# 20k/geodesic_raytracing

Measured on AMD Instinct MI355X. Metric: Mrays/sec at 3840x2160 Kerr (whole frame: prepass + init + adaptive Verlet + render-data + anisotropic render), higher is better.
Workload: dtype f32; 1 GPU; kerr_boyer (Boyer-Lindquist rs=1 a=0.45) 3840x2160, camera (0,0,-4,0) fov 90, adaptive_sampling off, prepass on, tol 1e-06, background 4096x2048 RGBA8 10 mips, anisotropy 8; mode=fused, prepass_lookahead=True, prepass_lookahead_depth=1, frames_in_flight=3, prepass=look-ahead on side streams, priming_frames=0, build_key=c7636d8b88329620-v80s8, counters_tag=kerr_a045_4k, program=substituted (parameters baked in, metric_manager.hpp:153-166), parallelism=single GPU

## Files before the change

### geodesic_raytracing_amd/__init__.py

```python
import ctypes
import os

_HERE = os.path.dirname(os.path.abspath(__file__))
LIB_PATH = os.path.join(_HERE, "libgeodesic_hip.so")

if not os.path.exists(LIB_PATH):
    raise ImportError(
        f"{LIB_PATH} is missing: build it with `python -c 'import __graft_entry__ as g; g.build()'` "
        "(there is no CPU fallback for the ray kernels)")

lib = ctypes.CDLL(LIB_PATH)

c_void_p = ctypes.c_void_p
c_int = ctypes.c_int
c_float = ctypes.c_float
c_char_p = ctypes.c_char_p
c_size_t = ctypes.c_size_t


class Features(ctypes.Structure):
    _fields_ = [
        ("adaptive_sampling_threshold", c_float), ("field_of_view", c_float), ("max_acceleration_change", c_float),
        ("max_precision_radius", c_float), ("min_step", c_float), ("ray_skip", c_float), ("universe_size", c_float),
        ("adaptive_sampling", c_int), ("redshift", c_int), ("reparameterisation", c_int), ("use_old_redshift", c_int),
# ... 64 lines not shown
                ("block_rows", c_int), ("strip_rank", c_int), ("strip_count", c_int), ("termination_buffer", c_void_p),
                ("prepass_width", c_int), ("prepass_height", c_int), ("e0", c_void_p), ("e1", c_void_p), ("e2", c_void_p),
                ("e3", c_void_p), ("cfg", c_void_p), ("dfg", c_void_p), ("attempt_counter", c_void_p), ("tile_order", c_void_p),
                ("waves_per_simd", c_int), ("shading", TraceShading), ("lattice", c_int), ("pending_only", c_int), ("inline_prepass", c_int),
                ("tile_cost", c_void_p), ("tile_order_by_history", c_int), ("lattice_rays", c_void_p), ("parking", ParkingLot), ("speculative_classes", c_int), ("guessed", c_void_p)]


class Transport(ctypes.Structure):
    GROUP = ctypes.CFUNCTYPE(c_int, c_void_p)
    SEND = ctypes.CFUNCTYPE(c_int, c_void_p, c_void_p, c_size_t, c_int, c_void_p)
    RECV = ctypes.CFUNCTYPE(c_int, c_void_p, c_void_p, c_size_t, c_int, c_void_p)
    _fields_ = [("user", c_void_p), ("group_begin", GROUP), ("group_end", GROUP), ("send", SEND), ("recv", RECV)]


MODE_REFERENCE, MODE_FUSED = 0, 1
EVAL_METRIC_TENSOR, EVAL_METRIC_DERIVATIVES, EVAL_ACCELERATION, EVAL_TO_POLAR, EVAL_FROM_POLAR, EVAL_ORIGIN_DISTANCE = range(6)
(STAGE_CAMERA, STAGE_PREPASS, STAGE_INIT, STAGE_TRACE, STAGE_RENDER_DATA, STAGE_ADAPTIVE, STAGE_RENDER) = range(7)
STAGE_NAMES = ["camera", "prepass", "init", "trace", "render_data", "adaptive", "render"]
(BUF_RAYS_IN, BUF_RAYS_COUNT, BUF_RENDER_DATA, BUF_TERMINATION, BUF_CAMERA_GENERIC, BUF_TETRAD0, BUF_TETRAD1, BUF_TETRAD2,
 BUF_TETRAD3, BUF_RAYS_ADAPTIVE, BUF_RAYS_ADAPTIVE_COUNT, BUF_CFG, BUF_DFG, BUF_CAMERA_QUAT) = range(14)

_SIGNATURES = {
    "gr_last_error": (c_char_p, []),
    "gr_features_default": (None, [ctypes.POINTER(Features)]),
    "gr_metric_builtin": (c_int, [c_char_p, ctypes.POINTER(c_void_p)]),
    "gr_metric_load_script": (c_int, [c_char_p, c_char_p, ctypes.POINTER(c_void_p)]),
    "gr_metric_from_info": (c_int, [ctypes.POINTER(MetricInfo), ctypes.POINTER(c_char_p), ctypes.POINTER(c_float), ctypes.POINTER(c_void_p)]),
    "gr_metric_destroy": (None, [c_void_p]),
    "gr_metric_get_info": (c_int, [c_void_p, ctypes.POINTER(MetricInfo)]),
    "gr_metric_dynamic_var_name": (c_char_p, [c_void_p, c_int]),
    "gr_metric_dynamic_var_default": (c_float, [c_void_p, c_int]),
    "gr_metric_argument_string": (c_int, [c_void_p, ctypes.POINTER(Features), c_int, ctypes.POINTER(c_float), c_int,
                                          c_char_p, c_size_t, ctypes.POINTER(c_size_t)]),
    "gr_metric_substituted_op_counts": (c_int, [c_void_p, ctypes.POINTER(c_float), c_int, ctypes.POINTER(c_int), ctypes.POINTER(c_int),
                                                ctypes.POINTER(c_int)]),
    "gr_metric_evaluate_count": (c_int, [c_int]),
    "gr_metric_evaluate": (c_int, [c_void_p, c_int, ctypes.POINTER(ctypes.c_double), ctypes.POINTER(ctypes.c_double), ctypes.POINTER(c_float), c_int,
                                   ctypes.POINTER(ctypes.c_double), c_int]),
    "gr_program_create": (c_int, [c_char_p, c_int, ctypes.POINTER(c_void_p)]),
    "gr_program_complete": (c_int, [c_void_p]),
    "gr_program_precompile_frame_path": (c_int, [c_char_p]),
    "gr_program_precompile": (c_int, [c_char_p]),
    "gr_program_create_async": (c_int, [c_char_p, c_int, ctypes.POINTER(c_void_p)]),
    "gr_program_future_poll": (c_int, [c_void_p, ctypes.POINTER(c_void_p)]),
    "gr_program_future_destroy": (None, [c_void_p]),
    "gr_program_destroy": (None, [c_void_p]),
    "gr_program_manager_create": (c_int, [c_void_p, c_int, ctypes.POINTER(Features), ctypes.POINTER(c_float), c_int, ctypes.POINTER(c_void_p)]),
    "gr_program_manager_update": (c_int, [c_void_p, ctypes.POINTER(Features), ctypes.POINTER(c_float), c_int]),
    "gr_program_manager_current": (c_int, [c_void_p, c_int, ctypes.POINTER(c_void_p), ctypes.POINTER(c_int)]),
    "gr_program_manager_dynamic": (c_void_p, [c_void_p]),
    "gr_program_manager_destroy": (None, [c_void_p]),
    "gr_do_generic_rays_scheduled": (c_int, [c_void_p, c_void_p, c_void_p, c_void_p, c_int, c_void_p, c_void_p, c_void_p, c_void_p, c_void_p]),
    "gr_sort_tiles_by_cost": (c_int, [c_void_p, c_void_p, c_void_p, c_int, c_int, c_void_p, c_void_p]),
    "gr_program_manager_counters": (None, [c_void_p, ctypes.POINTER(ctypes.c_ulonglong)]),
    "gr_program_kernel_info": (c_int, [c_void_p, c_char_p, ctypes.POINTER(c_int), ctypes.POINTER(c_int), ctypes.POINTER(c_int)]),
    "gr_cart_to_generic": (c_int, [c_void_p, c_void_p, c_void_p, c_void_p, c_int, c_float, c_void_p]),
    "gr_init_basis_vectors": (c_int, [c_void_p, c_void_p, c_void_p, c_int, ctypes.POINTER(c_float), c_void_p, c_void_p,
                                      c_void_p, c_void_p, c_void_p]),
    "gr_clear_termination_buffer": (c_int, [c_void_p, c_void_p, c_void_p, c_int, c_int]),
    "gr_init_rays_generic": (c_int, [c_void_p, c_void_p, c_void_p, c_void_p, c_void_p, c_void_p, c_int, c_int, c_void_p, c_int,
                                     c_int, c_int, c_void_p, c_void_p, c_void_p, c_void_p, c_void_p, c_void_p, c_int, c_int]),
    "gr_tiled_slot_count": (c_int, [c_int, c_int]),
    "gr_do_generic_rays": (c_int, [c_void_p, c_void_p, c_void_p, c_void_p, c_int, c_void_p, c_void_p, c_void_p, c_void_p, c_int,
                                   c_int, c_int, c_int, c_void_p, c_void_p, c_int, c_void_p]),
    "gr_calculate_singularities": (c_int, [c_void_p, c_void_p, c_void_p, c_void_p, c_int, c_void_p, c_int, c_int]),
    "gr_calculate_render_data": (c_int, [c_void_p, c_void_p, c_void_p, c_void_p, c_int, c_void_p, c_void_p, c_int, c_int,
# ... 134 lines not shown
```

### geodesic_raytracing_amd/csrc/capi.cpp

```cpp
#include "../../include/geodesic_hip_internal.h"

#include <dlfcn.h>
#include <hip/hip_runtime_api.h>
#include <hip/hiprtc.h>
#include <sys/stat.h>
#include <unistd.h>

#include <chrono>
#include <cmath>
#include <cstdio>
#include <algorithm>
#include <atomic>
#include <cstdlib>
#include <cstring>
#include <fstream>
#include <map>
#include <memory>
#include <condition_variable>
#include <mutex>
#include <sstream>
#include <string>
#include <system_error>
#include <thread>
#include <vector>
// ... 669 lines not shown
        env[vel_names[i]] = velocity ? velocity[i] : 0.0;
    }
    for (size_t i = 0; i < m->vars.names.size(); i++)
        env["cfg->" + m->vars.names[i]] = cfg_values ? (double)cfg_values[i] : (double)m->vars.defaults[i];
    env["always_lightlike"] = 0.0;
    const gr::MetricImpl& impl = m->desc.raw;
    auto eval_all = [&](const std::vector<sym::E>& v, double* dst) { for (size_t i = 0; i < v.size(); i++) dst[i] = sym::eval(v[i], env); };
    switch (what) {
        case GR_EVAL_METRIC_TENSOR:
            for (int i = 0; i < 16; i++) out[i] = 0.0;
            if (impl.real_eq.size() == 4) { for (int i = 0; i < 4; i++) out[i * 4 + i] = sym::eval(impl.real_eq[(size_t)i], env); }
            else eval_all(impl.real_eq, out);
            break;
        case GR_EVAL_METRIC_DERIVATIVES:
            for (int i = 0; i < 64; i++) out[i] = 0.0;
            if (impl.derivatives.size() == 16) { for (int k = 0; k < 4; k++) for (int i = 0; i < 4; i++) out[k * 16 + i * 4 + i] = sym::eval(impl.derivatives[(size_t)(k * 4 + i)], env); }
            else eval_all(impl.derivatives, out);
            break;
        case GR_EVAL_ACCELERATION: eval_all(impl.accel, out); break;
        case GR_EVAL_TO_POLAR: eval_all(impl.to_polar, out); break;
        case GR_EVAL_FROM_POLAR: eval_all(impl.from_polar, out); break;
        case GR_EVAL_ORIGIN_DISTANCE: {
            double polar[4];
            eval_all(impl.to_polar, polar);
            for (int i = 0; i < 4; i++) env[pos_names[i]] = polar[i];
            out[0] = sym::eval(impl.distance_function, env);
            break;
        }
    }
    return GR_OK;
    GR_TRY_END
}

int gr_metric_substituted_op_counts(const gr_metric* m, const float* cfg_values, int num_cfg_values, int* accel_ops,
                                    int* accel_transcendentals, int* coord_ops) {
    if (!m) return fail(GR_ERROR_INVALID_ARGUMENT, "null metric");
    if (m->settings_only) return fail(GR_ERROR_INVALID_ARGUMENT, "a metric made by gr_metric_from_info has no expressions to count");
    GR_TRY_BEGIN
    std::vector<float> vals(cfg_values, cfg_values + (cfg_values ? num_cfg_values : 0));
    const gr::MetricImpl concrete = m->desc.concrete(m->vars.substitution(vals));
    const sym::OpCount accel = sym::count_ops(concrete.accel);
    std::vector<sym::E> coord = concrete.to_polar;
    coord.push_back(concrete.distance_function);
    if (accel_ops) *accel_ops = accel.ops;
    if (accel_transcendentals) *accel_transcendentals = accel.transcendental;
    if (coord_ops) *coord_ops = sym::count_ops(coord).ops;
    return GR_OK;
    GR_TRY_END
}

int gr_argument_string_accelerations_call_trig(const char* argument_string) {
    if (!argument_string) return -1;
    std::vector<std::string> opts;
    for (auto& tok : split_arguments(argument_string))
        if (tok.rfind("-D", 0) == 0) opts.push_back(tok);
    return accelerations_without_trig(opts) ? 0 : 1;
}

int gr_program_precompile(const char* argument_string) {
    if (!argument_string) return fail(GR_ERROR_INVALID_ARGUMENT, "null argument string");
    std::string code, rest, setup;
    int rc = compile_code_object(argument_string, code);
    if (rc != GR_OK) return rc;
    rc = compile_code_object(argument_string, rest, nullptr, PART_REST);
    if (rc != GR_OK) return rc;
    return compile_setup_module(argument_string, setup);
// ... 990 lines not shown
```

### geodesic_raytracing_amd/csrc/metric_codegen.cpp

```cpp
#include <functional>
#include <unordered_set>
#include "metric_codegen.hpp"

#include <cmath>
#include <cstdio>
#include <cstring>
#include <sstream>
#include <iomanip>
#include <stdexcept>

using namespace sym;

namespace gr {


static bool parse_bool(const std::string& v) { return v == "true" || v == "1"; }

void MetricConfig::apply(const std::map<std::string, std::string>& kv) {
    for (auto& [key, value] : kv) {
        if (key == "name") name = value;
        else if (key == "description") description = value;
        else if (key == "use_prepass") use_prepass = parse_bool(value);
        else if (key == "max_acceleration_change") max_acceleration_change = std::stof(value);
        else if (key == "singular") singular = parse_bool(value);
        else if (key == "traversable_event_horizon") traversable_event_horizon = parse_bool(value);
        else if (key == "singular_terminator") singular_terminator = std::stof(value);
        else if (key == "adaptive_precision") adaptive_precision = parse_bool(value);
        else if (key == "detect_singularities") detect_singularities = parse_bool(value);
        else if (key == "follow_geodesics_forward") follow_geodesics_forward = parse_bool(value);
        else if (key == "coordinate_system") {
            if (value == "X_Y_THETA_PHI") system = CoordinateSystem::X_Y_THETA_PHI;
            else if (value == "CARTESIAN") system = CoordinateSystem::CARTESIAN;
            else if (value == "CYLINDRICAL") system = CoordinateSystem::CYLINDRICAL;
            else system = CoordinateSystem::OTHER;
        }
        else if (key == "to_polar") to_polar = value;
        else if (key == "from_polar") from_polar = value;
// ... 306 lines not shown

std::string FeatureConfig::dynamic_argument_string() const {
    std::string fl, bl;
    for (auto& [name, val] : features) {
        if (val.index() == 0) bl += name + ",";
        else fl += name + ",";
    }
    std::string s = "-DKERNEL_IS_DYNAMIC ";
    if (!fl.empty()) { fl.pop_back(); s += "-DDYNAMIC_FLOAT_FEATURES=" + fl + " "; }
    if (!bl.empty()) { bl.pop_back(); s += "-DDYNAMIC_BOOL_FEATURES=" + bl + " "; }
    return s;
}

std::string FeatureConfig::static_argument_string() const {
    std::string s = "-DKERNEL_IS_STATIC ";
    for (auto& [name, val] : features)
        if (val.index() == 1) s += "-DFEATURE_" + name + "=" + float_literal(std::get<1>(val)) + " ";
    for (auto& [name, val] : features)
        if (val.index() == 0) s += "-DFEATURE_" + name + "=" + (std::get<0>(val) ? "1" : "0") + " ";
    return s;
}

std::vector<unsigned char> FeatureConfig::pack() const {
    std::vector<unsigned char> buf;
    auto push = [&](const void* p) {
        const unsigned char* c = (const unsigned char*)p;
        buf.insert(buf.end(), c, c + 4);
    };
    for (auto& [name, val] : features)
        if (val.index() == 1) { float f = std::get<1>(val); push(&f); }
    for (auto& [name, val] : features)
        if (val.index() == 0) { int i = std::get<0>(val) ? 1 : 0; push(&i); }
    return buf;
}


std::string build_argument_string(const MetricDescriptor& desc, const MetricImpl& impl_in,
                                  const MetricConfig& cfg, const DynamicVars& vars, bool is_static,
                                  const FeatureConfig& features, bool linear_framebuffer) {
    MetricImpl impl = impl_in;
    {
        std::unordered_map<E, E> memo;
        for (auto* v : {&impl.real_eq, &impl.derivatives, &impl.accel})
            for (auto& e : *v) e = share_reciprocals(e, memo);
    }
    std::vector<E> scoped;
    scoped.insert(scoped.end(), impl.real_eq.begin(), impl.real_eq.end());
    scoped.insert(scoped.end(), impl.derivatives.begin(), impl.derivatives.end());
    scoped.insert(scoped.end(), impl.accel.begin(), impl.accel.end());
    Temporaries temps = hoist_position_temporaries(scoped);
    const auto* names = &temps.names;

    std::string s;
    if (linear_framebuffer) s += "-DLINEAR_FRAMEBUFFER ";
    s += "-DRS_IMPL=1 -DC_IMPL=1 ";

    for (size_t i = 0; i < impl.real_eq.size(); i++)
        s += "-DF" + std::to_string(i + 1) + "_I=" + to_c(impl.real_eq[i], names) + " ";

    bool constant_theta = cfg.system == CoordinateSystem::X_Y_THETA_PHI && desc.is_spherical;

    if (impl.derivatives.size() == 16) {
        for (int j = 0; j < 4; j++)
            for (int i = 0; i < 4; i++)
                s += "-DF" + std::to_string(j * 4 + i + 1) + "_P=" + to_c(impl.derivatives[i * 4 + j], names) + " ";
    } else {
// ... 88 lines not shown
                }
                if (!ok) sums_only = false;
            }
            walk(e->a); walk(e->b); walk(e->s);
        };
        for (E r : everything) walk(r);
        tanh_in_sums_only = any_tanh && sums_only;
        if (tanh_in_sums_only) s += "-DGR_TANH_IN_SUMS_ONLY ";
    }

    if (!vars.names.empty()) {
        std::string v;
        for (auto& n : vars.names) v += n + ",";
        v.pop_back();
        s += "-DDYNVARS=" + v + " ";
    }

    {
        Fn4 c2p = [](E t, E x, E y, E z) -> std::vector<E> {
            E r = fn1(F_SQRT, add(add(mul(x, x), mul(y, y)), mul(z, z)));
            E theta = fn2(F_ATAN2, fn1(F_SQRT, add(mul(x, x), mul(y, y))), z);
            E phi = fn2(F_ATAN2, y, x);
            return {t, r, theta, phi};
        };
        std::vector<E> full, d;
        total_diff(c2p, full, d);
        for (int i = 0; i < 4; i++) s += "-DCART_TO_POL" + std::to_string(i) + "=" + to_c(full[i]) + " ";
        for (int i = 0; i < 4; i++) s += "-DCART_TO_POL_D" + std::to_string(i) + "=" + to_c(d[i]) + " ";
    }

    for (int i = 0; i < 4; i++) s += "-DGEO_ACCEL" + std::to_string(i) + "=" + to_c(impl.accel[i], names) + " ";
    if (is_static) {
        bool lowered_differs = false;
        const std::vector<E> lowered = sym::lower_for_device(impl.accel, tanh_in_sums_only, &lowered_differs);
        bool any_negation = false;
        for (E a : lowered) any_negation |= a->op == sym::NEG;
        if (lowered_differs || any_negation) {
            const Temporaries device_temps = hoist_position_temporaries(lowered, "qv");
            std::string t;
            for (auto& [name, e] : device_temps.defs) t += name + "=" + sym::to_c_negations_pushed(e, &device_temps.names, true) + ",";
            if (t.empty()) t = "qv_unused=0.0f,";
            t.pop_back();
            s += "-DGR_DEVICE_TEMPORARIES=" + t + " ";
            for (int i = 0; i < 4; i++) s += "-DGR_DEVICE_ACCEL" + std::to_string(i) + "=" + sym::to_c_negations_pushed(lowered[i], &device_temps.names) + " ";
        }
    }
    for (int i = 0; i < 4; i++) s += "-DFIX_LIGHT" + std::to_string(i) + "=" + to_c(impl.fix_light[i]) + " ";
    s += "-DMETRIC_TIME_G00=" + to_c(impl.real_eq[0], names) + " ";

    if (temps.defs.empty()) {
        s += "-DTEMPORARIES0=DUMMY ";
    } else {
        std::string t;
        for (auto& [name, e] : temps.defs) t += name + "=" + to_c(e, names, true) + ",";
        t.pop_back();
        s += "-DTEMPORARIES0=" + t + " ";
        std::unordered_map<E, std::string> cfg_names;
        std::function<void(E)> wrap_leaves = [&](E e) {
            if (!e || cfg_names.count(e)) return;
            if (e->op == VAR) { cfg_names.emplace(e, "gm::cfgf(" + e->name + ")"); return; }
            wrap_leaves(e->a); wrap_leaves(e->b); wrap_leaves(e->s);
        };
        std::string c, p;
        for (auto& [name, e] : temps.defs) {
            if (e->deps == sym::DEP_CFG) {
                wrap_leaves(e);
                c += "c" + name + "=gm::cfgf(" + to_c(e, &cfg_names, true) + "),";
// ... 20 lines not shown
```

### geodesic_raytracing_amd/csrc/metric_codegen.hpp

```cpp
#pragma once
#include <functional>
#include <map>
#include <string>
#include <variant>
#include <vector>

#include "sym.hpp"

namespace gr {

enum class CoordinateSystem { X_Y_THETA_PHI, CARTESIAN, CYLINDRICAL, OTHER };

struct MetricConfig {
    std::string name;
    std::string description;
    bool use_prepass = false;
    float max_acceleration_change = 0.0000001f;
    bool singular = false;
    bool traversable_event_horizon = false;
    float singular_terminator = 1;
    bool adaptive_precision = true;
    bool detect_singularities = false;
    bool follow_geodesics_forward = false;
    bool has_cylindrical_singularity = false;
// ... 31 lines not shown

struct MetricImpl {
    std::vector<sym::E> accel, fix_light, real_eq, derivatives;
    std::vector<sym::E> to_polar, dt_to_spherical, from_polar, dt_from_spherical;
    sym::E distance_function = nullptr;
    std::vector<sym::E> coordinate_periodicity;
};

struct MetricDescriptor {
    MetricImpl raw;
    bool is_big = false;
    bool is_spherical = false;
    sym::OpCount accel_ops;
    sym::OpCount coord_ops;

    void load(const MetricFunctions& f, const MetricConfig& cfg);
    MetricImpl concrete(const std::map<std::string, sym::E>& substitution) const;
};

struct FeatureConfig {
    std::map<std::string, std::variant<bool, float>> features;
    void set(const std::string& n, bool v) { features[n] = v; }
    void set(const std::string& n, float v) { features[n] = v; }
    static FeatureConfig defaults();
    std::string dynamic_argument_string() const;
    std::string static_argument_string() const;
    std::vector<unsigned char> pack() const;
};

std::string build_argument_string(const MetricDescriptor& desc, const MetricImpl& impl,
                                  const MetricConfig& cfg, const DynamicVars& vars, bool is_static,
                                  const FeatureConfig& features, bool linear_framebuffer = true);

std::string float_literal(float v);

}
```

### geodesic_raytracing_amd/csrc/sym.cpp

```cpp
#include "sym.hpp"

#include <algorithm>
#include <cmath>
#include <cstdio>
#include <cstring>
#include <deque>
#include <functional>
#include <mutex>
#include <stdexcept>
#include <unordered_set>

namespace sym {

namespace {

struct Key {
    Op op;
    Fn fn;
    uint64_t cbits;
    std::string name;
    uint32_t a, b, s;
    bool operator==(const Key& o) const {
        return op == o.op && fn == o.fn && cbits == o.cbits && a == o.a && b == o.b && s == o.s &&
               name == o.name;
    }
};
struct KeyHash {
    size_t operator()(const Key& k) const {
        uint64_t h = 1469598103934665603ull;
        auto mix = [&](uint64_t v) {
            h ^= v + 0x9e3779b97f4a7c15ull + (h << 6) + (h >> 2);
        };
        mix(k.op);
        mix(k.fn);
        mix(k.cbits);
        mix(std::hash<std::string>()(k.name));
        mix(k.a);
        mix(k.b);
        mix(k.s);
        return (size_t)h;
// ... 885 lines not shown
    std::function<bool(E)> delicate = [&](E e) -> bool {
        if (!e || e->op == CONST || e->op == VAR) return false;
        auto it = delicate_memo.find(e);
        if (it != delicate_memo.end()) return it->second;
        bool d = e->op == DIV || e->op == FN1 || (e->op == FN2 && !is_cmp(e->fn)) || delicate(e->a) || delicate(e->b) || delicate(e->s);
        delicate_memo.emplace(e, d);
        return d;
    };
    std::unordered_set<E> forced;
    auto parameter_only = [](E e) { return e && e->deps == DEP_CFG; };
    for (E e : order) {
        if (parameter_only(e)) continue;
        for (E c : {e->a, e->b, e->s})
            if (parameter_only(c) && delicate(c)) forced.insert(c);
    }
    for (E r : roots)
        if (parameter_only(r) && delicate(r)) forced.insert(r);

    Temporaries t;
    const uint32_t pos_mask = DEP_V1 | DEP_V2 | DEP_V3 | DEP_V4 | DEP_CFG;
    for (E e : order) {
        if (e->op == CONST || e->op == VAR) continue;
        if (e->deps & ~pos_mask) continue;
        if (e->deps == 0) continue;
        if (refs[e] < 2 && !forced.count(e)) continue;
        if (e->op == NEG && (e->a->op == VAR || e->a->op == CONST)) continue;
        std::string name = prefix + std::to_string(t.defs.size());
        t.defs.emplace_back(name, e);
        t.names.emplace(e, name);
    }
    return t;
}


Cx cx(E re) { return Cx{re, constant(0.0)}; }
Cx cx(E re, E im) { return Cx{re, im}; }
Cx cadd(Cx a, Cx b) { return Cx{add(a.re, b.re), add(a.im, b.im)}; }
Cx csub(Cx a, Cx b) { return Cx{sub(a.re, b.re), sub(a.im, b.im)}; }
Cx cneg(Cx a) { return Cx{neg(a.re), neg(a.im)}; }
Cx cconj(Cx a) { return Cx{a.re, neg(a.im)}; }
Cx cmul(Cx a, Cx b) {
    return Cx{sub(mul(a.re, b.re), mul(a.im, b.im)), add(mul(a.re, b.im), mul(a.im, b.re))};
}
E cabs2(Cx a) { return add(mul(a.re, a.re), mul(a.im, a.im)); }
E cabs(Cx a) {
    if (is_zero(a.im)) return fn1(F_FABS, a.re);
    if (is_zero(a.re)) return fn1(F_FABS, a.im);
    return fn1(F_SQRT, cabs2(a));
}
Cx cdiv(Cx a, Cx b) {
    if (is_zero(b.im)) return Cx{div(a.re, b.re), div(a.im, b.re)};
    E d = cabs2(b);
    Cx n = cmul(a, cconj(b));
    return Cx{div(n.re, d), div(n.im, d)};
}
Cx cpowi(Cx a, int n) {
    if (n == 0) return cx(constant(1.0));
    if (n < 0) return cdiv(cx(constant(1.0)), cpowi(a, -n));
    Cx r = a;
    for (int i = 1; i < n; i++) r = cmul(r, a);
    return r;
}
Cx csqrt_real(E a) {
    if (a->op == CONST) {
        if (a->c >= 0) return cx(constant(std::sqrt(a->c)));
        return Cx{constant(0.0), constant(std::sqrt(-a->c))};
// ... 20 lines not shown
```

### geodesic_raytracing_amd/csrc/sym.hpp

```cpp
#pragma once
#include <cstdint>
#include <map>
#include <string>
#include <unordered_map>
#include <vector>

namespace sym {

enum Op : uint8_t { CONST, VAR, ADD, SUB, MUL, DIV, NEG, FN1, FN2, SELECT };

enum Fn : uint8_t {
    F_SIN, F_COS, F_TAN, F_ASIN, F_ACOS, F_ATAN, F_EXP, F_LOG, F_SQRT, F_FABS, F_SINH, F_COSH,
    F_TANH, F_SIGN,
    F_EXP2_FAST, F_RSQRT_FAST,
    F_ATAN2, F_POW, F_FMOD, F_MIN, F_MAX,
    F_CSQRT_RE, F_CSQRT_IM,
    F_LT, F_LE, F_EQ, F_GT, F_GE,
    F_NONE,
    F_SIN2, F_COS2, F_SINCOS
};

struct Node {
    Op op;
    Fn fn;
// ... 14 lines not shown
    DEP_IV = 1u << 4,
    DEP_DV = 1u << 5,
    DEP_CFG = 1u << 6,
    DEP_OTHER = 1u << 7
};

E constant(double v);
E var(const std::string& name);
E add(E a, E b);
E sub(E a, E b);
E mul(E a, E b);
E div(E a, E b);
E neg(E a);
E fn1(Fn f, E a);
E fn2(Fn f, E a, E b);
E select(E cond, E if_true, E if_false);
E powi(E a, int n);

inline bool is_const(E e) { return e->op == CONST; }
inline bool is_zero(E e) { return e->op == CONST && e->c == 0.0; }
inline bool is_one(E e) { return e->op == CONST && e->c == 1.0; }

E diff(E e, const std::string& wrt);
E subst(E e, const std::map<std::string, E>& m);
double eval(E e, const std::map<std::string, double>& env);

E cancel_round_trip(E e);
bool contains_division_or_angle(E e);

E share_reciprocals(E e, std::unordered_map<E, E>& memo);

std::vector<E> lower_for_device(const std::vector<E>& roots, bool fast_tanh, bool* changed);

std::string to_c(E e, const std::unordered_map<E, std::string>* names = nullptr, bool is_definition = false);
std::string to_c_negations_pushed(E e, const std::unordered_map<E, std::string>* names = nullptr, bool is_definition = false);
std::string const_to_c(double v);

struct OpCount { int ops = 0; int transcendental = 0; };
OpCount count_ops(const std::vector<E>& roots);

struct Temporaries {
    std::vector<std::pair<std::string, E>> defs;
    std::unordered_map<E, std::string> names;
};
Temporaries hoist_position_temporaries(const std::vector<E>& roots, const std::string& prefix = "pv");

struct Cx {
    E re, im;
};
Cx cx(E re);
Cx cx(E re, E im);
Cx cadd(Cx a, Cx b);
Cx csub(Cx a, Cx b);
Cx cmul(Cx a, Cx b);
Cx cdiv(Cx a, Cx b);
Cx cneg(Cx a);
Cx cconj(Cx a);
Cx cpowi(Cx a, int n);
Cx csqrt_principal(Cx a);
Cx csqrt_real(E a);
E cabs2(Cx a);
E cabs(Cx a);
Cx csin(Cx a);
Cx ccos(Cx a);

}
// ... 1 lines not shown
```

### include/geodesic_hip_internal.h

```cpp
#ifndef GEODESIC_HIP_INTERNAL_H
#define GEODESIC_HIP_INTERNAL_H

#include "geodesic_hip.h"

#ifdef __cplusplus
extern "C" {
#endif

struct gr_frame_tuning {
    int ray_compaction;
    int rays_per_lane;
    int fused_shading;
    int inline_prepass;
    int trace_waves_per_simd;
    int tile_history;
    int park_lanes;
    int park_trips;
    int next_strip_rank;
    int next_strip_rank2;
    float next_geodesic_time, next_geodesic_time2;
    int count_attempts;
    int guess_still_camera;
    int reuse_still_camera;
    int speculative_classes;
};
void gr_frame_tuning_default(gr_frame_tuning* out);

enum { GR_GEOBUF_PATH = 0, GR_GEOBUF_VELOCITY = 1, GR_GEOBUF_DS = 2, GR_GEOBUF_COUNT = 3, GR_GEOBUF_TRANSPORTED0 = 4,
       GR_GEOBUF_TRANSPORTED1 = 5, GR_GEOBUF_TRANSPORTED2 = 6, GR_GEOBUF_TRANSPORTED3 = 7 };
void* gr_geodesic_camera_buffer(gr_geodesic_camera* g, int which);

enum { GR_BUF_RAYS_IN = 0, GR_BUF_RAYS_COUNT = 1, GR_BUF_RENDER_DATA = 2, GR_BUF_TERMINATION = 3, GR_BUF_CAMERA_GENERIC = 4,
       GR_BUF_TETRAD0 = 5, GR_BUF_TETRAD1 = 6, GR_BUF_TETRAD2 = 7, GR_BUF_TETRAD3 = 8, GR_BUF_RAYS_ADAPTIVE = 9,
       GR_BUF_RAYS_ADAPTIVE_COUNT = 10, GR_BUF_CFG = 11, GR_BUF_DFG = 12, GR_BUF_CAMERA_QUAT = 13 };
void* gr_render_state_buffer(gr_render_state* s, int which);

void gr_program_manager_counters(const gr_program_manager* pm, unsigned long long out[4]);

typedef struct gr_program_future gr_program_future;
int gr_program_create_async(const char* argument_string, int device, gr_program_future** out);
int gr_program_precompile_frame_path(const char* argument_string);
int gr_program_future_poll(gr_program_future* f, gr_program** out);
void gr_program_future_destroy(gr_program_future* f);


int gr_metric_substituted_op_counts(const gr_metric* m, const float* cfg_values, int num_cfg_values, int* accel_ops,
                                    int* accel_transcendentals, int* coord_ops);


int gr_program_kernel_info(const gr_program* p, const char* kernel_name, int* vgprs, int* sgprs, int* scratch_bytes);

int gr_render_strips(gr_program* p, void* stream, const void* render_data, void* out_rgba_f32,
                     const void* background1, const void* background2, int bg_width, int bg_height, int bg_levels,
                     int width, int height, int block_rows, int strip_rank, int strip_count, int compact_out,
                     int max_probes, const void* cfg, const void* dfg);
int gr_strip_local_blocks(int height, int block_rows, int strip_rank, int strip_count);


int gr_prepass_fused(gr_program* p, void* stream, const void* camera_generic, const void* camera_quat,
                     void* termination_buffer, int prepass_width, int prepass_height,
                     const void* e0, const void* e1, const void* e2, const void* e3,
                     const void* cfg, const void* dfg);
int gr_prepass_fused_strips(gr_program* p, void* stream, const void* camera_generic, const void* camera_quat,
                            void* termination_buffer, int prepass_width, int prepass_height,
                            const void* e0, const void* e1, const void* e2, const void* e3, const void* cfg, const void* dfg,
                            int image_height, int block_rows, int strip_rank, int strip_count, void* cell_attempts, int row_margin);

int gr_camera_prepass(gr_program* p, void* stream, const void* position_cart, float flip, const float basis_speed[3],
                      void* position_generic_out, void* e0_out, void* e1_out, void* e2_out, void* e3_out, const void* camera_quat,
                      void* termination_buffer, int prepass_width, int prepass_height, const void* cfg, const void* dfg,
                      int image_height, int block_rows, int strip_rank, int strip_count, void* cell_attempts, int row_margin);

long long gr_tile_order_bytes(int width, int height, int block_rows, int strip_rank, int strip_count);
int gr_order_tiles(gr_program* p, void* stream, const void* termination_buffer, const void* cell_attempts, int prepass_width,
                   int prepass_height, int width, int height, int block_rows, int strip_rank, int strip_count, void* tile_order);
int gr_do_generic_rays_scheduled(gr_program* p, void* stream, void* rays, const void* ray_count, int tile_count, const void* cfg, const void* dfg,
                                 void* attempt_counter, const void* tile_order, void* tile_cost);
int gr_sort_tiles_by_cost(gr_program* p, void* stream, const void* tile_cost, int tiles_x, int tiles_y, void* tile_order, void* work);

int gr_order_tiles_by_history(gr_program* p, void* stream, const void* tile_history, int width, int height, int block_rows,
                              int strip_rank, int strip_count, void* tile_order, int shift_x, int shift_y);
// ... 115 lines not shown
```

Baseline: 1972 Mrays/s.

## Factor shared position-only denominators in baked geodesic acceleration expressions

Adds a symbolic rational-polynomial factoring pass that rewrites the baked acceleration expressions so they share common factored denominators, cutting reciprocals in the Verlet integrator's inner loop. Each rewritten component is checked numerically against the original on sampled states, including points near the pole, near the horizon and far out, for equivalence and f32 accuracy. A rewrite is kept only if a simple cycle model predicts fewer cycles. It risks larger numerators, different f32 rounding, and extra host compile time, and can be disabled with an environment variable.

```diff
diff --git a/geodesic_raytracing_amd/__init__.py b/geodesic_raytracing_amd/__init__.py
--- a/geodesic_raytracing_amd/__init__.py
+++ b/geodesic_raytracing_amd/__init__.py
@@ -120,6 +120,7 @@
     "gr_metric_dynamic_var_default": (c_float, [c_void_p, c_int]),
     "gr_metric_argument_string": (c_int, [c_void_p, ctypes.POINTER(Features), c_int, ctypes.POINTER(c_float), c_int,
                                           c_char_p, c_size_t, ctypes.POINTER(c_size_t)]),
+    "gr_device_algebra_last_report": (c_int, [ctypes.POINTER(ctypes.c_double), ctypes.POINTER(c_int), ctypes.POINTER(c_int)]),
     "gr_metric_substituted_op_counts": (c_int, [c_void_p, ctypes.POINTER(c_float), c_int, ctypes.POINTER(c_int), ctypes.POINTER(c_int),
                                                 ctypes.POINTER(c_int)]),
     "gr_metric_evaluate_count": (c_int, [c_int]),
diff --git a/geodesic_raytracing_amd/csrc/capi.cpp b/geodesic_raytracing_amd/csrc/capi.cpp
--- a/geodesic_raytracing_amd/csrc/capi.cpp
+++ b/geodesic_raytracing_amd/csrc/capi.cpp
@@ -725,6 +725,14 @@
     GR_TRY_END
 }
 
+int gr_device_algebra_last_report(double* cycles, int* counts, int* flags) {
+    const gr::DeviceAlgebraReport& r = gr::last_device_algebra_report();
+    if (cycles) { cycles[0] = r.before_cycles; cycles[1] = r.after_cycles; }
+    if (counts) for (int k = 0; k < 5; k++) { counts[k] = r.before[k]; counts[5 + k] = r.after[k]; }
+    if (flags) for (int i = 0; i < 4; i++) { flags[i] = r.equal[i]; flags[4 + i] = r.accurate[i]; flags[8 + i] = r.taken[i]; }
+    return GR_OK;
+}
+
 int gr_metric_substituted_op_counts(const gr_metric* m, const float* cfg_values, int num_cfg_values, int* accel_ops,
                                     int* accel_transcendentals, int* coord_ops) {
     if (!m) return fail(GR_ERROR_INVALID_ARGUMENT, "null metric");
diff --git a/geodesic_raytracing_amd/csrc/metric_codegen.cpp b/geodesic_raytracing_amd/csrc/metric_codegen.cpp
--- a/geodesic_raytracing_amd/csrc/metric_codegen.cpp
+++ b/geodesic_raytracing_amd/csrc/metric_codegen.cpp
@@ -3,6 +3,8 @@
 #include "metric_codegen.hpp"
 
 #include <cmath>
+#include <cstdlib>
+#include <random>
 #include <cstdio>
 #include <cstring>
 #include <sstream>
@@ -375,6 +377,119 @@
     for (auto& [name, val] : features)
         if (val.index() == 0) { int i = std::get<0>(val) ? 1 : 0; push(&i); }
     return buf;
+}
+
+thread_local DeviceAlgebraReport g_device_algebra_report;
+const DeviceAlgebraReport& last_device_algebra_report() { return g_device_algebra_report; }
+
+static std::vector<E> device_algebra(const std::vector<E>& today, const MetricConfig& cfg) {
+    DeviceAlgebraReport& report = g_device_algebra_report;
+    report = DeviceAlgebraReport();
+    report.before_cycles = sym::model_cycles(today, &report.before[0], &report.before[1], &report.before[2], &report.before[3], &report.before[4]);
+    report.after_cycles = report.before_cycles;
+    for (int k = 0; k < 5; k++) report.after[k] = report.before[k];
+    const char* off = std::getenv("GR_NO_DEVICE_ALGEBRA");
+    if (cfg.system != CoordinateSystem::X_Y_THETA_PHI || (off && *off && std::strcmp(off, "0") != 0)) return today;
+    int rewritten = 0;
+    std::vector<E> candidate = sym::factor_device_denominators(today, &rewritten);
+    if (rewritten == 0) return today;
+
+    std::mt19937_64 rng(20261016);
+    std::uniform_real_distribution<double> u(0.0, 1.0);
+    auto uni = [&](double lo, double hi) { return lo + (hi - lo) * u(rng); };
+    std::vector<std::map<std::string, double>> states;
+    auto state = [&](double r, double theta) {
+        std::map<std::string, double> env;
+        env["v1"] = uni(-1, 1); env["v2"] = r; env["v3"] = theta; env["v4"] = uni(-3, 3);
+        const double far = std::max(1.0, r);
+        env["iv1"] = uni(-1, 1); env["iv2"] = uni(-1, 1); env["iv3"] = uni(-1, 1) / far; env["iv4"] = uni(-1, 1) / far;
+        for (auto& [k, v] : env) v = (double)(float)v;
+        states.push_back(env);
+    };
+    for (int i = 0; i < 48; i++) state(uni(1.5, 30.0), uni(0.05, M_PI - 0.05));
+    for (double theta : {1e-2, 1e-3, 1e-4, M_PI - 1e-3}) state(uni(2.0, 10.0), theta);
+    for (double r : {1e2, 1e3, 1e4, 1e5}) state(r, uni(0.1, M_PI - 0.1));
+    {
+        std::vector<E> dens;
+        std::unordered_set<E> seen;
+        std::function<void(E)> walk = [&](E e) {
+            if (!e || e->op == CONST || e->op == VAR || !seen.insert(e).second) return;
+            if (e->op == DIV && (e->b->deps & ~(DEP_V1 | DEP_V2 | DEP_V3 | DEP_V4 | DEP_CFG)) == 0 && (e->b->deps & DEP_V2)) dens.push_back(e->b);
+            walk(e->a); walk(e->b); walk(e->s);
+        };
+        for (E r : today) walk(r);
+        for (E d : dens) {
+            const double theta = uni(0.2, M_PI - 0.2);
+            std::map<std::string, double> env{{"v1", 0.0}, {"v3", theta}, {"v4", 0.0}, {"iv1", 0.0}, {"iv2", 0.0}, {"iv3", 0.0}, {"iv4", 0.0}};
+            auto f = [&](double r) { env["v2"] = r; try { return sym::eval(d, env); } catch (...) { return std::nan(""); } };
+            double root = -1, prev = f(50.0);
+            for (double r = 50.0; r > 1e-3; r *= 0.98) {
+                const double now = f(r);
+                if (std::isfinite(now) && std::isfinite(prev) && (now < 0) != (prev < 0)) {
+                    double lo = r, hi = r / 0.98;
+                    for (int k = 0; k < 80; k++) { const double mid = 0.5 * (lo + hi); ((f(mid) < 0) == (now < 0) ? lo : hi) = mid; }
+                    root = hi;
+                    break;
+                }
+                prev = now;
+            }
+            if (root > 0)
+                for (double eps : {1e-2, 1e-3, 1e-4}) state(root * (1 + eps), theta);
+        }
+    }
+
+    const double ulp = std::ldexp(1.0, -24);
+    std::vector<E> chosen = today;
+    for (size_t i = 0; i < today.size(); i++) {
+        if (candidate[i] == today[i]) continue;
+        bool equal = true;
+        double worst_old = 0, worst_new = 0, sum_old = 0, sum_new = 0;
+        int counted = 0;
+        try {
+            for (auto& env : states) {
+                const double a = sym::eval(today[i], env), b = sym::eval(candidate[i], env);
+                if (!std::isfinite(a) || !std::isfinite(b)) { equal = std::isfinite(a) == std::isfinite(b); if (!equal) break; continue; }
+                if (std::fabs(a - b) > 1e-6 * std::max(std::fabs(a), std::fabs(b))) { equal = false; break; }
+                const char* iv[4] = {"iv1", "iv2", "iv3", "iv4"};
+                double vel[4], diag[4], size = 0;
+                std::map<std::string, double> unit = env;
+                for (int k = 0; k < 4; k++) { vel[k] = env.at(iv[k]); unit[iv[k]] = 0.0; }
+                for (int k = 0; k < 4; k++) { unit[iv[k]] = 1.0; diag[k] = sym::eval(today[i], unit); unit[iv[k]] = 0.0; size += std::fabs(diag[k] * vel[k] * vel[k]); }
+                for (int k = 0; k < 4; k++)
+                    for (int l = k + 1; l < 4; l++) {
+                        unit[iv[k]] = 1.0; unit[iv[l]] = 1.0;
+                        size += std::fabs((sym::eval(today[i], unit) - diag[k] - diag[l]) * vel[k] * vel[l]);
+                        unit[iv[k]] = 0.0; unit[iv[l]] = 0.0;
+                    }
+                if (!(size > 0) || !std::isfinite(size)) continue;
+                const double eo = std::fabs((double)sym::eval_f32(today[i], env) - a) / size;
+                const double en = std::fabs((double)sym::eval_f32(candidate[i], env) - a) / size;
+                if (!std::isfinite(en) && std::isfinite(eo)) { equal = false; break; }
+                worst_old = std::max(worst_old, eo); worst_new = std::max(worst_new, en);
+                sum_old += eo; sum_new += en;
+                counted++;
+            }
+        } catch (const std::exception&) {
+            equal = false;
+        }
+        const bool accurate = counted > 0 && worst_new <= worst_old + ulp && sum_new <= sum_old + ulp * counted;
+        report.accurate[i] = accurate;
+        report.equal[i] = equal;
+        if (equal && accurate) chosen[i] = candidate[i];
+    }
+    for (size_t i = 0; i < today.size(); i++) {
+        if (chosen[i] == today[i]) continue;
+        std::vector<E> without = chosen;
+        without[i] = today[i];
+        if (sym::model_cycles(without) <= sym::model_cycles(chosen)) chosen = without;
+    }
+    int counts[5];
+    const double after = sym::model_cycles(chosen, &counts[0], &counts[1], &counts[2], &counts[3], &counts[4]);
+    if (!(after < report.before_cycles)) return today;
+    report.after_cycles = after;
+    for (int k = 0; k < 5; k++) report.after[k] = counts[k];
+    for (size_t i = 0; i < today.size(); i++) report.taken[i] = chosen[i] != today[i];
+    return chosen;
 }
 
 
@@ -529,7 +644,12 @@
     for (int i = 0; i < 4; i++) s += "-DGEO_ACCEL" + std::to_string(i) + "=" + to_c(impl.accel[i], names) + " ";
     if (is_static) {
         bool lowered_differs = false;
-        const std::vector<E> lowered = sym::lower_for_device(impl.accel, tanh_in_sums_only, &lowered_differs);
+        std::vector<E> lowered = sym::lower_for_device(impl.accel, tanh_in_sums_only, &lowered_differs);
+        {
+            const std::vector<E> factored = device_algebra(lowered, cfg);
+            lowered_differs |= factored != lowered;
+            lowered = factored;
+        }
         bool any_negation = false;
         for (E a : lowered) any_negation |= a->op == sym::NEG;
         if (lowered_differs || any_negation) {
diff --git a/geodesic_raytracing_amd/csrc/metric_codegen.hpp b/geodesic_raytracing_amd/csrc/metric_codegen.hpp
--- a/geodesic_raytracing_amd/csrc/metric_codegen.hpp
+++ b/geodesic_raytracing_amd/csrc/metric_codegen.hpp
@@ -87,6 +87,13 @@
                                   const MetricConfig& cfg, const DynamicVars& vars, bool is_static,
                                   const FeatureConfig& features, bool linear_framebuffer = true);
 
+struct DeviceAlgebraReport {
+    double before_cycles = 0, after_cycles = 0;
+    int before[5] = {0, 0, 0, 0, 0}, after[5] = {0, 0, 0, 0, 0};
+    bool equal[4] = {false, false, false, false}, accurate[4] = {false, false, false, false}, taken[4] = {false, false, false, false};
+};
+const DeviceAlgebraReport& last_device_algebra_report();
+
 std::string float_literal(float v);
 
 }
diff --git a/geodesic_raytracing_amd/csrc/sym.cpp b/geodesic_raytracing_amd/csrc/sym.cpp
--- a/geodesic_raytracing_amd/csrc/sym.cpp
+++ b/geodesic_raytracing_amd/csrc/sym.cpp
@@ -6,6 +6,7 @@
 #include <cstring>
 #include <deque>
 #include <functional>
+#include <map>
 #include <mutex>
 #include <stdexcept>
 #include <unordered_set>
@@ -957,6 +958,438 @@
     return t;
 }
 
+namespace {
+typedef std::vector<int> Mono;
+typedef std::map<Mono, double> Poly;
+
+struct Algebra {
+    std::vector<E> atom_node;
+    std::vector<int> atom_kind;
+    std::vector<int> atom_partner;
+    std::unordered_map<E, int> atom_of;
+
+    struct Factor { Poly p; E node; int atom; };
+    std::vector<Factor> factors;
+    std::map<int, int> atom_factor;
+
+    struct Rat { Poly num; std::map<int, int> den; };
+    std::unordered_map<E, std::pair<bool, Rat>> memo;
+
+    static constexpr size_t kMaxTerms = 400;
+    static constexpr int kMaxDenominator = 8;
+    static bool position_only(E e) { return (e->deps & ~(DEP_V1 | DEP_V2 | DEP_V3 | DEP_V4 | DEP_CFG)) == 0; }
+
+    int atom(E node, int kind, int partner = -1) {
+        auto it = atom_of.find(node);
+        if (it != atom_of.end()) return it->second;
+        atom_node.push_back(node);
+        atom_kind.push_back(kind);
+        atom_partner.push_back(partner);
+        atom_of.emplace(node, (int)atom_node.size() - 1);
+        return (int)atom_node.size() - 1;
+    }
+    static Mono trim(Mono m) { while (!m.empty() && m.back() == 0) m.pop_back(); return m; }
+    static int exp_of(const Mono& m, int a) { return a < (int)m.size() ? m[a] : 0; }
+    static Mono with(Mono m, int a, int delta) {
+        if ((int)m.size() <= a) m.resize(a + 1, 0);
+        m[a] += delta;
+        return trim(m);
+    }
+    void add_term(Poly& p, const Mono& m, double c) {
+        if (c == 0.0) return;
+        for (int a = 0; a < (int)m.size(); a++)
+            if (atom_kind[a] == 2 && m[a] >= 2) {
+                const Mono rest = with(m, a, -2);
+                const int s = atom_partner[a];
+                add_term(p, with(rest, s, 1), c);
+                add_term(p, with(rest, s, 2), -c);
+                return;
+            }
+        double& v = p[m];
+        v += c;
+        if (v == 0.0) p.erase(m);
+    }
+    Poly padd(const Poly& a, const Poly& b, double sb = 1.0) {
+        Poly r = a;
+        for (auto& [m, c] : b) add_term(r, m, sb * c);
+        return r;
+    }
+    Poly pmul(const Poly& a, const Poly& b) {
+        Poly r;
+        for (auto& [ma, ca] : a)
+            for (auto& [mb, cb] : b) {
+                Mono m(std::max(ma.size(), mb.size()), 0);
+                for (size_t i = 0; i < ma.size(); i++) m[i] += ma[i];
+                for (size_t i = 0; i < mb.size(); i++) m[i] += mb[i];
+                add_term(r, trim(m), ca * cb);
+            }
+        return r;
+    }
+    static Poly pconst(double c) { Poly p; if (c != 0.0) p[Mono()] = c; return p; }
+    static Poly patom(int a) { Poly p; p[with(Mono(), a, 1)] = 1.0; return p; }
+    static double scale(const Poly& p) { double s = 0; for (auto& t : p) s = std::max(s, std::fabs(t.second)); return s; }
+    static bool is_constant(const Poly& p) { return p.empty() || (p.size() == 1 && p.begin()->first.empty()); }
+    static double constant_of(const Poly& p) { return p.empty() ? 0.0 : p.begin()->second; }
+
+    int factor_of_atom(int a) {
+        auto it = atom_factor.find(a);
+        if (it != atom_factor.end()) return it->second;
+        factors.push_back(Factor{patom(a), atom_node[a], a});
+        atom_factor.emplace(a, (int)factors.size() - 1);
+        return (int)factors.size() - 1;
+    }
+
+    bool divide(const Poly& p, const Factor& f, Poly& q) {
+        q.clear();
+        if (f.atom >= 0) {
+            for (auto& [m, c] : p) {
+                if (exp_of(m, f.atom) < 1) return false;
+                q[with(m, f.atom, -1)] = c;
+            }
+            return true;
+        }
+        int v = -1, d = 0;
+        double lc = 0;
+        for (int a = 0; a < (int)atom_node.size(); a++) {
+            if (atom_kind[a] != 0) continue;
+            int da = 0;
+            for (auto& t : f.p) da = std::max(da, exp_of(t.first, a));
+            if (da <= d) continue;
+            int n = 0;
+            for (auto& t : f.p) if (exp_of(t.first, a) == da) n++;
+            auto lead = f.p.find(with(Mono(), a, da));
+            if (n == 1 && lead != f.p.end()) { v = a; d = da; lc = lead->second; }
+        }
+        if (v < 0) return false;
+        const double tol = 1e-9 * scale(p);
+        Poly r = p;
+        for (int guard = 0; guard < 4096; guard++) {
+            const Mono* lead = nullptr;
+            for (auto& t : r)
+                if (std::fabs(t.second) > tol && exp_of(t.first, v) >= d && (!lead || exp_of(t.first, v) > exp_of(*lead, v))) lead = &t.first;
+            if (!lead) break;
+            const Mono lm = *lead;
+            const Mono qm = with(lm, v, -d);
+            const double qc = r[lm] / lc;
+            add_term(q, qm, qc);
+            Poly t;
+            t[qm] = qc;
+            r = padd(r, pmul(t, f.p), -1.0);
+            r.erase(lm);
+            for (auto it = r.begin(); it != r.end();) it = std::fabs(it->second) <= 1e-15 * scale(p) ? r.erase(it) : std::next(it);
+        }
+        for (auto& t : r)
+            if (std::fabs(t.second) > tol) return false;
+        return true;
+    }
+
+    void factorize(Poly p, double& c, std::map<int, int>& exps, E self) {
+        c = 1.0;
+        if (p.empty()) return;
+        bool whole = true;
+        for (int a = 0; a < (int)atom_node.size(); a++) {
+            int lo = 1 << 30;
+            for (auto& t : p) lo = std::min(lo, exp_of(t.first, a));
+            if (lo > 0) {
+                Poly q;
+                for (auto& [m, cm] : p) q[with(m, a, -lo)] = cm;
+                p = q;
+                exps[factor_of_atom(a)] += lo;
+                whole = false;
+            }
+        }
+        for (int i = 0; i < (int)factors.size(); i++) {
+            if (factors[i].atom >= 0) continue;
+            Poly q;
+            while (!is_constant(p) && divide(p, factors[i], q)) { p = q; exps[i]++; whole = false; }
+        }
+        if (is_constant(p)) { c = constant_of(p); return; }
+        factors.push_back(Factor{p, self && whole ? self : to_node(p), -1});
+        exps[(int)factors.size() - 1]++;
+    }
+
+    E to_node(const Poly& p) {
+        E sum = constant(0.0);
+        for (auto& [m, c] : p) {
+            E term = constant(c);
+            for (int a = 0; a < (int)m.size(); a++)
+                if (m[a]) term = mul(term, powi(atom_node[a], m[a]));
+            sum = add(sum, term);
+        }
+        return sum;
+    }
+
+    Rat combine(const Rat& x, const Rat& y, double sy) {
+        Rat r;
+        r.den = x.den;
+        for (auto& [f, e] : y.den) r.den[f] = std::max(r.den[f], e);
+        auto lift = [&](const Rat& z) {
+            Poly p = z.num;
+            for (auto& [f, e] : r.den) {
+                auto it = z.den.find(f);
+                for (int k = it == z.den.end() ? 0 : it->second; k < e; k++) p = pmul(p, factors[f].p);
+            }
+            return p;
+        };
+        r.num = padd(lift(x), lift(y), sy);
+        return r;
+    }
+
+    bool rational(E e, Rat& out) {
+        auto it = memo.find(e);
+        if (it != memo.end()) { out = it->second.second; return it->second.first; }
+        bool ok = position_only(e);
+        Rat r;
+        if (ok) switch (e->op) {
+            case CONST: r.num = pconst(e->c); break;
+            case FN1:
+                if ((e->fn == F_SIN2 || e->fn == F_COS2 || e->fn == F_SINCOS) && (e->a->deps & ~DEP_CFG) != 0) {
+                    const int s = atom(fn1(F_SIN2, e->a), 1);
+                    if (e->fn == F_SIN2) r.num = patom(s);
+                    else if (e->fn == F_COS2) r.num = padd(pconst(1.0), patom(s), -1.0);
+                    else r.num = patom(atom(e, 2, s));
+                    break;
+                }
+                [[fallthrough]];
+            case VAR:
+            case FN2:
+            case SELECT: r.num = patom(atom(e, 0)); break;
+            case NEG: { Rat a; ok = rational(e->a, a); r = a; r.num = padd(Poly(), a.num, -1.0); break; }
+            case ADD:
+            case SUB: { Rat a, b; ok = rational(e->a, a) && rational(e->b, b); if (ok) r = combine(a, b, e->op == ADD ? 1.0 : -1.0); break; }
+            case MUL: {
+                Rat a, b;
+                ok = rational(e->a, a) && rational(e->b, b);
+                if (ok) { r.num = pmul(a.num, b.num); r.den = a.den; for (auto& [f, k] : b.den) r.den[f] += k; }
+                break;
+            }
+            case DIV: {
+                Rat a, b;
+                ok = rational(e->a, a) && rational(e->b, b);
+                if (!ok) break;
+                double c;
+                std::map<int, int> exps;
+                factorize(b.num, c, exps, b.den.empty() ? e->b : nullptr);
+                ok = c != 0.0;
+                r.num = pmul(a.num, pconst(1.0 / c));
+                for (auto& [f, k] : b.den)
+                    for (int i = 0; i < k; i++) r.num = pmul(r.num, factors[f].p);
+                r.den = a.den;
+                for (auto& [f, k] : exps) r.den[f] += k;
+                break;
+            }
+        }
+        int depth = 0;
+        for (auto& fk : r.den) depth += fk.second;
+        if (r.num.size() > kMaxTerms || depth > kMaxDenominator) ok = false;
+        memo.emplace(e, std::make_pair(ok, r));
+        out = r;
+        return ok;
+    }
+
+    void register_denominators(E e, std::unordered_set<E>& seen) {
+        if (!e || !seen.insert(e).second) return;
+        register_denominators(e->a, seen); register_denominators(e->b, seen); register_denominators(e->s, seen);
+        if (e->op != DIV || !position_only(e->b) || e->b->op == CONST) return;
+        Rat b;
+        if (!rational(e->b, b) || !b.den.empty()) return;
+        double c;
+        std::map<int, int> exps;
+        factorize(b.num, c, exps, e->b);
+    }
+};
+
+struct Refactor {
+    Algebra& alg;
+    int rewritten = 0;
+    std::unordered_map<E, E> memo;
+    E run(E e) {
+        if (e->op == CONST || e->op == VAR) return e;
+        auto it = memo.find(e);
+        if (it != memo.end()) return it->second;
+        E r = nullptr;
+        switch (e->op) {
+            case ADD: r = add(run(e->a), run(e->b)); break;
+            case SUB: r = sub(run(e->a), run(e->b)); break;
+            case MUL: r = mul(run(e->a), run(e->b)); break;
+            case NEG: r = neg(run(e->a)); break;
+            case FN1: r = fn1(e->fn, run(e->a)); break;
+            case FN2: r = fn2(e->fn, run(e->a), run(e->b)); break;
+            case SELECT: r = select(run(e->a), run(e->b), run(e->s)); break;
+            case DIV: r = quotient(e); break;
+            default: throw std::runtime_error("factor_device_denominators: bad op");
+        }
+        memo.emplace(e, r);
+        return r;
+    }
+    E quotient(E e) {
+        E n = run(e->a);
+        Algebra::Rat b;
+        if (!Algebra::position_only(e->b) || e->b->op == CONST || !alg.rational(e->b, b)) return div(n, run(e->b));
+        double c;
+        std::map<int, int> exps;
+        alg.factorize(b.num, c, exps, nullptr);
+        for (auto& [f, k] : b.den) exps[f] -= k;
+        int divides = 0;
+        E only = nullptr;
+        for (auto& [f, k] : exps) if (k > 0) { divides += k; only = alg.factors[f].node; }
+        bool negative_exp = false;
+        for (auto& [f, k] : exps) negative_exp |= k < 0;
+        if (c == 1.0 && divides == 1 && !negative_exp && only == e->b) return div(n, run(e->b));
+        E num = c == 1.0 ? n : mul(constant(1.0 / c), n);
+        E den = constant(1.0);
+        for (auto& [f, k] : exps) {
+            if (k > 0) den = mul(den, powi(alg.factors[f].node, k));
+            if (k < 0) num = mul(num, powi(alg.factors[f].node, -k));
+        }
+        rewritten++;
+        return is_one(den) ? num : div(num, den);
+    }
+};
+
+E share_product_denominator(E e, const std::unordered_map<E, E>& partner, std::unordered_map<E, E>& memo, int& shared) {
+    if (e->op == CONST || e->op == VAR) return e;
+    auto it = memo.find(e);
+    if (it != memo.end()) return it->second;
+    auto R = [&](E x) { return x ? share_product_denominator(x, partner, memo, shared) : x; };
+    E r;
+    switch (e->op) {
+        case ADD: r = add(R(e->a), R(e->b)); break;
+        case SUB: r = sub(R(e->a), R(e->b)); break;
+        case MUL: r = mul(R(e->a), R(e->b)); break;
+        case NEG: r = neg(R(e->a)); break;
+        case FN1: r = fn1(e->fn, R(e->a)); break;
+        case FN2: r = fn2(e->fn, R(e->a), R(e->b)); break;
+        case SELECT: r = select(R(e->a), R(e->b), R(e->s)); break;
+        case DIV: {
+            auto p = partner.find(e->b);
+            if (p != partner.end()) {
+                const E product = p->second;
+                const E other = product->a == e->b ? product->b : product->a;
+                r = div(mul(R(e->a), other), product);
+                shared++;
+            } else {
+                r = div(R(e->a), R(e->b));
+            }
+            break;
+        }
+        default: throw std::runtime_error("share_product_denominator: bad op");
+    }
+    memo.emplace(e, r);
+    return r;
+}
+}
+
+std::vector<E> factor_device_denominators(const std::vector<E>& roots, int* rewritten) {
+    Algebra alg;
+    std::unordered_set<E> seen;
+    for (E r : roots) alg.register_denominators(r, seen);
+    Refactor rf{alg};
+    std::vector<E> out;
+    for (E r : roots) out.push_back(rf.run(r));
+    std::unordered_set<E> dens;
+    std::function<void(E)> collect = [&](E e) {
+        if (!e || e->op == CONST || e->op == VAR || !seen.insert(e).second) return;
+        if (e->op == DIV && Algebra::position_only(e->b) && e->b->op != CONST) dens.insert(e->b);
+        collect(e->a); collect(e->b); collect(e->s);
+    };
+    seen.clear();
+    for (E r : out) collect(r);
+    std::unordered_map<E, E> partner;
+    for (E d : dens)
+        if (d->op == MUL && Algebra::position_only(d->a) && Algebra::position_only(d->b))
+            for (E x : {d->a, d->b})
+                if (dens.count(x) && x->op != CONST && !partner.count(x)) partner.emplace(x, d);
+    int shared = 0;
+    if (!partner.empty()) {
+        std::unordered_map<E, E> memo;
+        for (E& r : out) r = share_product_denominator(r, partner, memo, shared);
+    }
+    if (rewritten) *rewritten = rf.rewritten + shared;
+    return out;
+}
+
+double model_cycles(const std::vector<E>& roots, int* muls, int* fmas, int* adds, int* rcps, int* others) {
+    std::unordered_map<E, int> refs;
+    std::vector<E> order;
+    std::unordered_set<E> seen;
+    std::function<void(E)> visit = [&](E e) {
+        if (!e) return;
+        refs[e]++;
+        if (!seen.insert(e).second) return;
+        visit(e->a); visit(e->b); visit(e->s);
+        order.push_back(e);
+    };
+    for (E r : roots) visit(r);
+    int nm = 0, nf = 0, na = 0, nr = 0, no = 0;
+    std::unordered_set<E> reciprocal;
+    auto single_product = [&](E x) { return x->op == MUL && refs[x] == 1; };
+    std::unordered_set<E> fused;
+    for (E e : order) {
+        switch (e->op) {
+            case ADD:
+            case SUB:
+                if (single_product(e->a) && !fused.count(e->a)) { fused.insert(e->a); nf++; }
+                else if (single_product(e->b) && !fused.count(e->b)) { fused.insert(e->b); nf++; }
+                else na++;
+                break;
+            case MUL: nm++; break;
+            case DIV:
+                if (reciprocal.insert(e->b).second) nr++;
+                if (!(is_const(e->a) && std::fabs(e->a->c) == 1.0)) nm++;
+                break;
+            case FN1:
+                if (e->fn == F_FABS || e->fn == F_SIGN) no++;
+                else if (e->fn == F_SIN2 || e->fn == F_COS2 || e->fn == F_SINCOS) no += 2;
+                else nr++;
+                break;
+            case FN2:
+            case SELECT: no++; break;
+            default: break;
+        }
+    }
+    nm -= (int)fused.size();
+    if (muls) *muls = nm;
+    if (fmas) *fmas = nf;
+    if (adds) *adds = na;
+    if (rcps) *rcps = nr;
+    if (others) *others = no;
+    return 2.25 * (nm + nf + na + no) + 8.1 * nr;
+}
+
+namespace {
+float eval32_rec(E e, const std::map<std::string, double>& env, std::unordered_map<E, float>& memo) {
+    if (e->op == CONST) return (float)e->c;
+    auto it = memo.find(e);
+    if (it != memo.end()) return it->second;
+    float r = 0;
+    switch (e->op) {
+        case VAR: {
+            auto v = env.find(e->name);
+            if (v == env.end()) throw std::runtime_error("eval_f32: unbound variable " + e->name);
+            r = (float)v->second;
+            break;
+        }
+        case ADD: r = eval32_rec(e->a, env, memo) + eval32_rec(e->b, env, memo); break;
+        case SUB: r = eval32_rec(e->a, env, memo) - eval32_rec(e->b, env, memo); break;
+        case MUL: r = eval32_rec(e->a, env, memo) * eval32_rec(e->b, env, memo); break;
+        case DIV: r = eval32_rec(e->a, env, memo) / eval32_rec(e->b, env, memo); break;
+        case NEG: r = -eval32_rec(e->a, env, memo); break;
+        case FN1: r = (float)apply1(e->fn, eval32_rec(e->a, env, memo)); break;
+        case FN2: r = (float)apply2(e->fn, eval32_rec(e->a, env, memo), eval32_rec(e->b, env, memo)); break;
+        case SELECT: r = eval32_rec(e->a, env, memo) != 0.0f ? eval32_rec(e->b, env, memo) : eval32_rec(e->s, env, memo); break;
+        default: throw std::runtime_error("eval_f32: bad op");
+    }
+    memo.emplace(e, r);
+    return r;
+}
+}
+
+float eval_f32(E e, const std::map<std::string, double>& env) {
+    std::unordered_map<E, float> memo;
+    return eval32_rec(e, env, memo);
+}
+
 
 Cx cx(E re) { return Cx{re, constant(0.0)}; }
 Cx cx(E re, E im) { return Cx{re, im}; }
diff --git a/geodesic_raytracing_amd/csrc/sym.hpp b/geodesic_raytracing_amd/csrc/sym.hpp
--- a/geodesic_raytracing_amd/csrc/sym.hpp
+++ b/geodesic_raytracing_amd/csrc/sym.hpp
@@ -70,6 +70,11 @@
 
 std::vector<E> lower_for_device(const std::vector<E>& roots, bool fast_tanh, bool* changed);
 
+std::vector<E> factor_device_denominators(const std::vector<E>& roots, int* rewritten);
+double model_cycles(const std::vector<E>& roots, int* muls = nullptr, int* fmas = nullptr, int* adds = nullptr, int* rcps = nullptr,
+                    int* others = nullptr);
+float eval_f32(E e, const std::map<std::string, double>& env);
+
 std::string to_c(E e, const std::unordered_map<E, std::string>* names = nullptr, bool is_definition = false);
 std::string to_c_negations_pushed(E e, const std::unordered_map<E, std::string>* names = nullptr, bool is_definition = false);
 std::string const_to_c(double v);
diff --git a/include/geodesic_hip_internal.h b/include/geodesic_hip_internal.h
--- a/include/geodesic_hip_internal.h
+++ b/include/geodesic_hip_internal.h
@@ -47,6 +47,8 @@
 int gr_metric_substituted_op_counts(const gr_metric* m, const float* cfg_values, int num_cfg_values, int* accel_ops,
                                     int* accel_transcendentals, int* coord_ops);
 
+
+int gr_device_algebra_last_report(double* cycles, int* counts, int* flags);
 
 int gr_program_kernel_info(const gr_program* p, const char* kernel_name, int* vgprs, int* sgprs, int* scratch_bytes);
 
```

New measurement: 2038 Mrays/s, median of 6. 1.03x the previous value.
